# PreferredAI/PyBMF

Measured on AMD Instinct MI355X. Metric: MU iterations/sec (BinaryMF-Penalty, 100k x 20k Boolean, k=64), higher is better.
Workload: dtype i8 (bits x int8 digit planes on the integer MFMA, exact int32 accumulation); fp64 master factors and scalars; 1 GPU; BinaryMF-Penalty MU, 100000x20000 dense Boolean X, k=64, reg=1 growth=1.02, init normal+balance seed 2024; mae_pass=False, operands=i8x3, splits_xv=2, splits_xtu=11

## Files before the change

pybmf_amd/csrc/cover.hip:

```cpp
#include "common.h"

#include <algorithm>
#include <cstdlib>

namespace {

constexpr int RB = 8, NW = 8;
constexpr int CH = 256;

__global__ __launch_bounds__(512) void cover_kernel(const uint32_t* __restrict__ X, int64_t ldx, int64_t words,
                                                     const uint64_t* __restrict__ rowbits,
                                                     const uint32_t* __restrict__ colbits, int64_t ldcb, int kp,
                                                     int64_t rows_pad, int rows_per_block, int y_big, int rows_big,
                                                     unsigned long long* __restrict__ counts,
                                                     const int32_t* __restrict__ stop) {
    if (stop && *stop != 0) return;
    __shared__ __attribute__((aligned(16))) uint32_t vt[BMF_MAX_KP + 1][CH];
    const int lane = threadIdx.x & 63;
    const int wave = __builtin_amdgcn_readfirstlane(threadIdx.x >> 6);
    const int64_t w0 = (int64_t)blockIdx.x * CH;
    const int nw = (int)min((int64_t)CH, words - w0);

    {
        constexpr int PIECES = BMF_MAX_KP * CH / 4;
#pragma unroll
        for (int base = 0; base < PIECES; base += 4 * 512) {
            u32x4 v[4];
#pragma unroll
            for (int q = 0; q < 4; ++q) {
                const int p = base + q * 512 + threadIdx.x;
                const int l = p / (CH / 4), pw = (p % (CH / 4)) * 4;
                v[q] = (l < kp && pw < nw) ? *reinterpret_cast<const u32x4*>(colbits + (int64_t)l * ldcb + w0 + pw)
                                           : u32x4{0u, 0u, 0u, 0u};
            }
#pragma unroll
            for (int q = 0; q < 4; ++q) {
                const int p = base + q * 512 + threadIdx.x;
                *reinterpret_cast<u32x4*>(&vt[p / (CH / 4)][(p % (CH / 4)) * 4]) = v[q];
            }
        }
        if (threadIdx.x < CH / 4) *reinterpret_cast<u32x4*>(&vt[BMF_MAX_KP][threadIdx.x * 4]) = u32x4{0u, 0u, 0u, 0u};
    }
    __syncthreads();

    const int by = (int)blockIdx.y;
    const int64_t r0 = by < y_big ? (int64_t)by * rows_big : (int64_t)y_big * rows_big + (int64_t)(by - y_big) * rows_per_block;
    const int64_t r1 = min(r0 + (by < y_big ? rows_big : rows_per_block), rows_pad);
    if (r0 >= r1) return;
    const bool lane_on = 4 * lane < nw;
    unsigned tp = 0, fp = 0;
    const int nrows_wave = (int)((r1 - r0) / NW);
    const uint32_t* xw = X + (r0 + wave) * ldx + w0 + (lane_on ? 4 * lane : 0);
    const unsigned row_step = (unsigned)(NW * ldx);
    for (int g = 0; g < nrows_wave; g += 64) {
        const int jl = min(g + lane, nrows_wave - 1);
        const unsigned long long uvec = rowbits[r0 + wave + (int64_t)NW * jl];
        const unsigned uv_lo = (g + lane < nrows_wave) ? (unsigned)uvec : 0u;
        const unsigned uv_hi = (g + lane < nrows_wave) ? (unsigned)(uvec >> 32) : 0u;
        const int nj = min(64, nrows_wave - g);
        const uint32_t* xg = xw + (size_t)g * row_step;
        u32x4 x_cur[RB], x_nxt[RB];
#pragma unroll
        for (int b = 0; b < RB; ++b) x_cur[b] = *reinterpret_cast<const u32x4*>(xg + (size_t)b * row_step);
        for (int j0 = 0; j0 < nj; j0 += RB) {
            const int jn = (j0 + RB < nj) ? j0 + RB : j0;
#pragma unroll
            for (int b = 0; b < RB; ++b) x_nxt[b] = *reinterpret_cast<const u32x4*>(xg + (size_t)(jn + b) * row_step);
#pragma unroll
            for (int b = 0; b < RB; ++b) {
                unsigned ulo = __builtin_amdgcn_readlane(uv_lo, j0 + b);
                unsigned uhi = __builtin_amdgcn_readlane(uv_hi, j0 + b);
                if ((ulo | uhi) == 0u) continue;
                u32x4 pd = {0u, 0u, 0u, 0u};
                while (ulo | uhi) {
                    const int l0 = ulo ? __builtin_ctz(ulo) : BMF_MAX_KP;
                    ulo &= ulo - 1;
                    const int l1 = ulo ? __builtin_ctz(ulo) : BMF_MAX_KP;
                    ulo &= ulo - 1;
                    const int l2 = uhi ? 32 + __builtin_ctz(uhi) : BMF_MAX_KP;
                    uhi &= uhi - 1;
                    const int l3 = uhi ? 32 + __builtin_ctz(uhi) : BMF_MAX_KP;
                    uhi &= uhi - 1;
                    const u32x4 v0 = *reinterpret_cast<const u32x4*>(&vt[l0][4 * lane]);
                    const u32x4 v1 = *reinterpret_cast<const u32x4*>(&vt[l1][4 * lane]);
                    const u32x4 v2 = *reinterpret_cast<const u32x4*>(&vt[l2][4 * lane]);
                    const u32x4 v3 = *reinterpret_cast<const u32x4*>(&vt[l3][4 * lane]);
                    pd |= (v0 | v1) | (v2 | v3);
                }
                if (!lane_on) pd = u32x4{0u, 0u, 0u, 0u};
#pragma unroll
                for (int q = 0; q < 4; ++q) {
                    tp += __popc(x_cur[b][q] & pd[q]);
                    fp += __popc(~x_cur[b][q] & pd[q]);
                }
            }
#pragma unroll
            for (int b = 0; b < RB; ++b) x_cur[b] = x_nxt[b];
        }
    }
    __shared__ unsigned red[2][NW];
    tp = wave_sum(tp);
    fp = wave_sum(fp);
    if (lane == 0) { red[0][wave] = tp; red[1][wave] = fp; }
    __syncthreads();
    if (threadIdx.x < 2) {
        unsigned long long t = 0;
#pragma unroll
        for (int w = 0; w < NW; ++w) t += red[threadIdx.x][w];
        if (t) atomicAdd(&counts[threadIdx.x], t);
    }
}

template <int N4, int TW>
__global__ __launch_bounds__(1024) void cover_wide_kernel(const uint32_t* __restrict__ X, int64_t ldx, int64_t words, int chunk_words,
                                                           const uint64_t* __restrict__ rowbits, const uint32_t* __restrict__ colbits,
                                                           int64_t ldcb, int kp, int64_t rows_pad, int rows_per_block,
                                                           unsigned long long* __restrict__ counts, const int32_t* __restrict__ stop) {
    if (stop && *stop != 0) return;
    constexpr int CW = 256 * N4 + 64 * TW;
#ifndef BMF_COVER_RBW
#define BMF_COVER_RBW 2
#endif
    constexpr int NWV = 16, RBW = BMF_COVER_RBW;
    constexpr int NS = N4 + (TW ? 1 : 0);
    static_assert(BMF_MAX_KP * CW * 4 <= 160 * 1024 && (TW == 0 || TW == 2 || TW == 4) && NS >= 1, "chunk must fit the LDS");
    __shared__ __attribute__((aligned(16))) uint32_t vt[BMF_MAX_KP * CW];
    const int lane = threadIdx.x & 63;
    const int wave = __builtin_amdgcn_readfirstlane(threadIdx.x >> 6);
    const int64_t w0 = (int64_t)blockIdx.x * chunk_words;
    const int nw = (int)min((int64_t)min(CW, chunk_words), words - w0);

    {
        constexpr int PPC = CW / 4;
        constexpr int PIECES = BMF_MAX_KP * PPC;
        for (int base = 0; base < PIECES; base += 4 * 1024) {
            u32x4 v[4];
#pragma unroll
            for (int q = 0; q < 4; ++q) {
                const int p = base + q * 1024 + (int)threadIdx.x;
                const int l = p / PPC, pw = (p % PPC) * 4;
                v[q] = (p < PIECES && l < kp && pw < nw) ? *reinterpret_cast<const u32x4*>(colbits + (int64_t)l * ldcb + w0 + pw) : u32x4{0u, 0u, 0u, 0u};
            }
#pragma unroll
            for (int q = 0; q < 4; ++q) {
                const int p = base + q * 1024 + (int)threadIdx.x;
                if (p < PIECES) *reinterpret_cast<u32x4*>(&vt[4 * p]) = v[q];
            }
        }
    }
    __syncthreads();

    const int64_t r0 = (int64_t)blockIdx.y * rows_per_block;
    const int64_t r1 = min(r0 + rows_per_block, rows_pad);
    unsigned tp = 0, pp = 0;
    if (r0 < r1) {
        int soff[NS];
        bool son[NS];
#pragma unroll
        for (int sg = 0; sg < NS; ++sg) {
            const int wpl = (sg < N4) ? 4 : TW;
            const int o = 256 * sg + wpl * lane;
            son[sg] = o < nw;
            soff[sg] = son[sg] ? o : 0;
        }
        const int nrows_wave = (int)((r1 - r0) / NWV);
        const uint32_t* xw = X + (r0 + wave) * ldx + w0;
        const unsigned row_step = (unsigned)(NWV * ldx);
        for (int g = 0; g < nrows_wave; g += 64) {
            const int jl = min(g + lane, nrows_wave - 1);
            const unsigned long long uvec = rowbits[r0 + wave + (int64_t)NWV * jl];
            const unsigned uv_lo = (g + lane < nrows_wave) ? (unsigned)uvec : 0u;
            const unsigned uv_hi = (g + lane < nrows_wave) ? (unsigned)(uvec >> 32) : 0u;
            const int nj = min(64, nrows_wave - g);
            const uint32_t* xg = xw + (size_t)g * row_step;
            u32x4 x_cur[RBW][NS], x_nxt[RBW][NS];
            auto load_rows = [&](int j, u32x4 (&dst)[RBW][NS]) {
#pragma unroll
                for (int b = 0; b < RBW; ++b)
#pragma unroll
                    for (int sg = 0; sg < NS; ++sg) {
                        const uint32_t* p_ = xg + (size_t)(j + b) * row_step + soff[sg];
#ifdef BMF_COVER_PLAIN_LOADS
                        if (sg < N4 || TW == 4) dst[b][sg] = *reinterpret_cast<const u32x4*>(p_);
                        else {
                            const u32x2 t = *reinterpret_cast<const u32x2*>(p_);
                            dst[b][sg] = u32x4{t[0], t[1], 0u, 0u};
                        }
#else
                        if (sg < N4 || TW == 4) dst[b][sg] = __builtin_nontemporal_load(reinterpret_cast<const u32x4*>(p_));
                        else {
                            const u32x2 t = __builtin_nontemporal_load(reinterpret_cast<const u32x2*>(p_));
                            dst[b][sg] = u32x4{t[0], t[1], 0u, 0u};
                        }
#endif
                    }
            };
            load_rows(0, x_cur);
            for (int j0 = 0; j0 < nj; j0 += RBW) {
                const int jn = (j0 + RBW < nj) ? j0 + RBW : j0;
                load_rows(jn, x_nxt);
#pragma unroll
                for (int b = 0; b < RBW; ++b) {
                    const unsigned ulo = __builtin_amdgcn_readlane(uv_lo, j0 + b);
                    const unsigned uhi = __builtin_amdgcn_readlane(uv_hi, j0 + b);
                    unsigned long long u = ((unsigned long long)uhi << 32) | ulo;
                    if (u == 0ull) continue;
                    u32x4 pd[NS];
#pragma unroll
                    for (int sg = 0; sg < NS; ++sg) pd[sg] = u32x4{0u, 0u, 0u, 0u};
                    while (u) {
                        const int l0 = __builtin_ctzll(u);
                        u &= u - 1;
                        const int l1 = u ? __builtin_ctzll(u) : l0;
                        u &= u - 1;
                        const uint32_t* c0 = vt + l0 * CW;
                        const uint32_t* c1 = vt + l1 * CW;
#pragma unroll
                        for (int sg = 0; sg < NS; ++sg) {
                            if (sg < N4 || TW == 4) {
                                const u32x4 v0 = *reinterpret_cast<const u32x4*>(c0 + soff[sg]);
                                const u32x4 v1 = *reinterpret_cast<const u32x4*>(c1 + soff[sg]);
                                pd[sg] |= v0 | v1;
                            } else {
                                const u32x2 v0 = *reinterpret_cast<const u32x2*>(c0 + soff[sg]);
                                const u32x2 v1 = *reinterpret_cast<const u32x2*>(c1 + soff[sg]);
                                pd[sg][0] |= v0[0] | v1[0];
                                pd[sg][1] |= v0[1] | v1[1];
                            }
                        }
                    }
#pragma unroll
                    for (int sg = 0; sg < NS; ++sg) {
                        const int nq = (sg < N4 || TW == 4) ? 4 : 2;
#pragma unroll
                        for (int q = 0; q < 4; ++q)
                            if (q < nq) {
                                const unsigned pw_ = son[sg] ? pd[sg][q] : 0u;
                                tp += __popc(x_cur[b][sg][q] & pw_);
                                pp += __popc(pw_);
                            }
                    }
                }
#pragma unroll
                for (int b = 0; b < RBW; ++b)
#pragma unroll
                    for (int sg = 0; sg < NS; ++sg) x_cur[b][sg] = x_nxt[b][sg];
            }
        }
    }
    tp = wave_sum(tp);
    pp = wave_sum(pp);
    __syncthreads();
    if (lane == 0) { vt[wave] = tp; vt[NWV + wave] = pp; }
    __syncthreads();
    if (threadIdx.x < 2) {
        unsigned long long t = 0, a_ = 0;
#pragma unroll
        for (int w = 0; w < NWV; ++w) { t += vt[w]; a_ += vt[NWV + w]; }
        const unsigned long long val = threadIdx.x == 0 ? t : a_ - t;
        if (val) atomicAdd(&counts[threadIdx.x], val);
    }
}

__global__ __launch_bounds__(1024) void cover_delta_kernel(const uint32_t* __restrict__ X, int64_t ldx, int64_t words, int chunk_words,
                                                            const uint64_t* __restrict__ rowbits, const uint64_t* __restrict__ rowbits_prev,
                                                            const uint32_t* __restrict__ colbits, int64_t ldcb, int kp, int64_t rows_pad,
                                                            int rows_per_block, unsigned long long* __restrict__ counts,
                                                            const uint64_t* __restrict__ copy_src, uint64_t* __restrict__ copy_dst, int64_t copy_n,
                                                            const int32_t* __restrict__ stop) {
    if (stop && *stop != 0) return;
    constexpr int CW = 640, NWV = 16, NS = 3;
    __shared__ __attribute__((aligned(16))) uint32_t vt[BMF_MAX_KP * CW];
    const int lane = threadIdx.x & 63;
    const int wave = __builtin_amdgcn_readfirstlane(threadIdx.x >> 6);
    const int64_t w0 = (int64_t)blockIdx.x * chunk_words;
    const int nw = (int)min((int64_t)chunk_words, words - w0);
    const int64_t r0 = (int64_t)blockIdx.y * rows_per_block;
    const int64_t r1 = min(r0 + rows_per_block, rows_pad);

    if (copy_n > 0) {
        const int64_t nthreads = (int64_t)gridDim.x * gridDim.y * 1024;
        for (int64_t i = ((int64_t)blockIdx.y * gridDim.x + blockIdx.x) * 1024 + threadIdx.x; i < copy_n; i += nthreads) copy_dst[i] = copy_src[i];
    }

    unsigned long long need = 0ull;
    for (int64_t r = r0 + threadIdx.x; r < r1; r += 1024) {
        const unsigned long long a_ = rowbits[r], b_ = rowbits_prev[r];
        if (a_ != b_) need |= a_ | b_;
    }
    if (threadIdx.x < 2) vt[threadIdx.x] = 0u;
    __syncthreads();
    if (need) {
        atomicOr(&vt[0], (unsigned)need);
        atomicOr(&vt[1], (unsigned)(need >> 32));
    }
    __syncthreads();
    need = ((unsigned long long)vt[1] << 32) | vt[0];
    __syncthreads();
    if (need == 0ull) return;

    {
        constexpr int PPC = CW / 4;
        constexpr int PIECES = BMF_MAX_KP * PPC;
        const int nneed = __builtin_popcountll(need);
        if (nneed <= 12) {
            const int slot = (int)threadIdx.x / PPC, pw = ((int)threadIdx.x % PPC) * 4;
            u32x4 v[2];
            int col[2];
#pragma unroll
            for (int q = 0; q < 2; ++q) {
                unsigned long long m_ = need;
                for (int i = 0; i < 6 * q + slot && m_; ++i) m_ &= m_ - 1;
                col[q] = (slot < 6 && m_) ? __builtin_ctzll(m_) : -1;
                v[q] = (col[q] >= 0 && col[q] < kp && pw < nw) ? *reinterpret_cast<const u32x4*>(colbits + (int64_t)col[q] * ldcb + w0 + pw) : u32x4{0u, 0u, 0u, 0u};
            }
#pragma unroll
            for (int q = 0; q < 2; ++q)
                if (col[q] >= 0) *reinterpret_cast<u32x4*>(&vt[col[q] * CW + pw]) = v[q];
        } else {
            for (int base = 0; base < PIECES; base += 5 * 1024) {
                u32x4 v[5];
#pragma unroll
                for (int q = 0; q < 5; ++q) {
                    const int p = base + q * 1024 + (int)threadIdx.x;
                    const int l = p / PPC, pw = (p % PPC) * 4;
                    v[q] = (l < kp && pw < nw) ? *reinterpret_cast<const u32x4*>(colbits + (int64_t)l * ldcb + w0 + pw) : u32x4{0u, 0u, 0u, 0u};
                }
#pragma unroll
                for (int q = 0; q < 5; ++q) *reinterpret_cast<u32x4*>(&vt[4 * (base + q * 1024 + (int)threadIdx.x)]) = v[q];
            }
        }
    }
    __syncthreads();

    int soff[NS];
    bool son[NS];
#pragma unroll
    for (int sg = 0; sg < NS; ++sg) {
        const int o = 256 * sg + (sg < 2 ? 4 : 2) * lane;
        son[sg] = o < nw;
        soff[sg] = son[sg] ? o : 0;
    }
    const int nseg = (nw + 255) / 256;

    auto add_product = [&](unsigned long long u, u32x4 (&pd)[NS]) {
        while (u) {
            const int l0 = __builtin_ctzll(u);
            u &= u - 1;
            const int l1 = u ? __builtin_ctzll(u) : l0;
            u &= u - 1;
            const uint32_t* c0 = vt + l0 * CW;
            const uint32_t* c1 = vt + l1 * CW;
#pragma unroll
            for (int sg = 0; sg < NS; ++sg) {
                if (sg >= nseg) continue;
                if (sg < 2) {
                    pd[sg] |= *reinterpret_cast<const u32x4*>(c0 + soff[sg]) | *reinterpret_cast<const u32x4*>(c1 + soff[sg]);
                } else {
                    const u32x2 v0 = *reinterpret_cast<const u32x2*>(c0 + soff[sg]);
                    const u32x2 v1 = *reinterpret_cast<const u32x2*>(c1 + soff[sg]);
                    pd[sg][0] |= v0[0] | v1[0];
                    pd[sg][1] |= v0[1] | v1[1];
                }
            }
        }
#pragma unroll
        for (int sg = 0; sg < NS; ++sg)
            if (!son[sg]) pd[sg] = u32x4{0u, 0u, 0u, 0u};
    };

    constexpr int SCAN = 8;
    unsigned tpn = 0, tpo = 0, ppn = 0, ppo = 0;
    const int nrows = (int)(r1 - r0);
    const uint32_t* xb = X + r0 * ldx + w0;
    int rank0 = 0;
    for (int base = 0; base < nrows; base += 64 * SCAN) {
        unsigned long long un[SCAN], uo[SCAN];
#pragma unroll
        for (int g = 0; g < SCAN; ++g) {
            const int row = min(base + 64 * g + lane, nrows - 1);
            un[g] = rowbits[r0 + row];
            uo[g] = rowbits_prev[r0 + row];
        }
        int l_row = 0, l_nlo = 0, l_nhi = 0, l_olo = 0, l_ohi = 0, cnt = 0;
#pragma unroll
        for (int g = 0; g < SCAN; ++g) {
            const bool d_ = base + 64 * g < nrows && un[g] != uo[g];
            const unsigned long long mask = __ballot(d_);
            const int rk = rank0 + (int)__builtin_amdgcn_mbcnt_hi((unsigned)(mask >> 32), __builtin_amdgcn_mbcnt_lo((unsigned)mask, 0u));
            unsigned long long mine = __ballot(d_ && (rk & (NWV - 1)) == wave);
            rank0 += __builtin_popcountll(mask);
            while (mine) {
                const int j = __builtin_ctzll(mine);
                mine &= mine - 1;
                const bool slot = lane == cnt;
                l_row = slot ? base + 64 * g + j : l_row;
                l_nlo = slot ? __builtin_amdgcn_readlane((int)(unsigned)un[g], j) : l_nlo;
                l_nhi = slot ? __builtin_amdgcn_readlane((int)(unsigned)(un[g] >> 32), j) : l_nhi;
                l_olo = slot ? __builtin_amdgcn_readlane((int)(unsigned)uo[g], j) : l_olo;
                l_ohi = slot ? __builtin_amdgcn_readlane((int)(unsigned)(uo[g] >> 32), j) : l_ohi;
                ++cnt;
            }
        }
        if (cnt == 0) continue;
        u32x4 x_cur[NS], x_nxt[NS];
        auto load_row = [&](int t, u32x4 (&dst)[NS]) {
            const uint32_t* xr = xb + (int64_t)__builtin_amdgcn_readlane(l_row, t) * ldx;
#pragma unroll
            for (int sg = 0; sg < NS; ++sg) {
                dst[sg] = u32x4{0u, 0u, 0u, 0u};
                if (sg >= nseg) continue;
                if (sg < 2) dst[sg] = __builtin_nontemporal_load(reinterpret_cast<const u32x4*>(xr + soff[sg]));
                else {
                    const u32x2 v = __builtin_nontemporal_load(reinterpret_cast<const u32x2*>(xr + soff[sg]));
                    dst[sg] = u32x4{v[0], v[1], 0u, 0u};
                }
            }
        };
        load_row(0, x_cur);
        for (int t = 0; t < cnt; ++t) {
            load_row(t + 1 < cnt ? t + 1 : t, x_nxt);
            const unsigned wn_lo = __builtin_amdgcn_readlane(l_nlo, t), wn_hi = __builtin_amdgcn_readlane(l_nhi, t);
            const unsigned wo_lo = __builtin_amdgcn_readlane(l_olo, t), wo_hi = __builtin_amdgcn_readlane(l_ohi, t);
            const unsigned long long wn = ((unsigned long long)wn_hi << 32) | wn_lo, wo = ((unsigned long long)wo_hi << 32) | wo_lo;
            u32x4 pn[NS], po[NS];
#pragma unroll
            for (int sg = 0; sg < NS; ++sg) pn[sg] = u32x4{0u, 0u, 0u, 0u};
            add_product(wn & wo, pn);
#pragma unroll
            for (int sg = 0; sg < NS; ++sg) po[sg] = pn[sg];
            add_product(wn & ~wo, pn);
            add_product(wo & ~wn, po);
#pragma unroll
            for (int sg = 0; sg < NS; ++sg)
#pragma unroll
                for (int q = 0; q < 4; ++q) {
                    tpn += __popc(x_cur[sg][q] & pn[sg][q]);
                    tpo += __popc(x_cur[sg][q] & po[sg][q]);
                    ppn += __popc(pn[sg][q]);
                    ppo += __popc(po[sg][q]);
                }
#pragma unroll
            for (int sg = 0; sg < NS; ++sg) x_cur[sg] = x_nxt[sg];
        }
    }
    int tp = (int)wave_sum(tpn - tpo);
    int pp = (int)wave_sum(ppn - ppo);
    __syncthreads();
    if (lane == 0) { vt[wave] = (unsigned)tp; vt[NWV + wave] = (unsigned)pp; }
    __syncthreads();
    if (threadIdx.x < 2) {
        long long t = 0, a_ = 0;
#pragma unroll
        for (int w = 0; w < NWV; ++w) { t += (int)vt[w]; a_ += (int)vt[NWV + w]; }
        const long long val = threadIdx.x == 0 ? t : a_ - t;
        if (val) atomicAdd(&counts[threadIdx.x], (unsigned long long)val);
    }
}

__global__ __launch_bounds__(256) void product_bits_kernel(const uint64_t* __restrict__ rowbits, int64_t rows,
                                                            const uint32_t* __restrict__ colbits, int64_t ldcb, int64_t words,
                                                            uint32_t* __restrict__ out, int64_t ldo) {
    const int64_t total = rows * words;
    for (int64_t idx = (int64_t)blockIdx.x * 256 + threadIdx.x; idx < total; idx += (int64_t)gridDim.x * 256) {
        const int64_t row = idx / words, w = idx - row * words;
        unsigned long long u = rowbits[row];
        unsigned pd = 0u;
        while (u) {
            const int l = __builtin_ctzll(u);
            u &= u - 1;
            pd |= colbits[(int64_t)l * ldcb + w];
        }
        out[row * ldo + w] = pd;
    }
}

__global__ __launch_bounds__(256) void confusion_rows_kernel(const uint32_t* __restrict__ G, int64_t ldg,
                                                              const uint32_t* __restrict__ P, int64_t ldp, int64_t rows,
                                                              int64_t words, uint32_t* __restrict__ tp,
                                                              uint32_t* __restrict__ fp) {
    const int lane = threadIdx.x & 63;
    const int64_t nwaves = (int64_t)gridDim.x * 4;
    for (int64_t r = (int64_t)blockIdx.x * 4 + (threadIdx.x >> 6); r < rows; r += nwaves) {
        unsigned a = 0u, b = 0u;
        for (int64_t w = lane; w < words; w += 64) {
            const uint32_t g = G[r * ldg + w], p = P[r * ldp + w];
            a += __popc(g & p);
            b += __popc(~g & p);
        }
        a = wave_sum(a);
        b = wave_sum(b);
        if (lane == 0) {
            tp[r] = a;
            fp[r] = b;
        }
    }
}

}

extern "C" int bmf_confusion_rows(const uint32_t* Gbits, int64_t ldg, const uint32_t* Pbits, int64_t ldp, int64_t rows,
                                  int64_t words, uint32_t* tp, uint32_t* fp, void* stream) {
    BMF_REQUIRE(Gbits && Pbits && tp && fp, "bmf_confusion_rows: null pointer");
    BMF_REQUIRE(rows >= 1 && words >= 1 && ldg >= words && ldp >= words, "bmf_confusion_rows: bad shape");
    const int64_t blocks = (rows + 3) / 4;
    BMF_LAUNCH(confusion_rows_kernel, dim3((unsigned)(blocks < 4096 ? blocks : 4096)), dim3(256), 0, (hipStream_t)stream, Gbits, ldg,
               Pbits, ldp, rows, words, tp, fp);
    BMF_LAUNCH_CHECK();
    return BMF_OK;
}

namespace {
template <int N4, int TW>
void launch_cover_wide(dim3 grid, hipStream_t s, const uint32_t* Xbits, int64_t ldx, int64_t words, int chunk_words, const uint64_t* rowbits,
                       const uint32_t* colbits, int64_t ldcb, int kp, int64_t rows_pad, int rows_per_block, unsigned long long* counts,
                       const int32_t* stop) {
    BMF_LAUNCH((cover_wide_kernel<N4, TW>), grid, dim3(1024), 0, s, Xbits, ldx, words, chunk_words, rowbits, colbits, ldcb, kp, rows_pad,
               rows_per_block, counts, stop);
}
}

int bmf_cover_launch(const uint32_t* Xbits, int64_t rows_pad, int64_t ldx, int64_t words, const uint64_t* rowbits,
                     const uint32_t* colbits, int64_t ldcb, int kp, unsigned long long* counts, const int32_t* stop,
                     hipStream_t s) {
    if (words >= 128) {
        const int chunks_w = (int)((words + 639) / 640);
        int cw = (int)(((words + chunks_w - 1) / chunks_w + 127) / 128 * 128);
        const int n4 = cw / 256 > 2 ? 2 : cw / 256, rem = cw - 256 * n4;
        const int tw = rem == 0 ? 0 : (rem <= 128 ? 2 : 4);
        const int cus = bmf_cu_count_current();
        int64_t groups = cus / chunks_w > 0 ? cus / chunks_w : 1;
        const int64_t units = rows_pad / 64;
        if (groups > units) groups = units;
        const int rows_per_block = (int)(((units + groups - 1) / groups) * 64);
        groups = (rows_pad + rows_per_block - 1) / rows_per_block;
        dim3 grid((unsigned)chunks_w, (unsigned)groups);
        bool launched = false;
#define BMF_CW_CASE(N4_, TW_) \
    if (n4 == N4_ && tw == TW_) { launch_cover_wide<N4_, TW_>(grid, s, Xbits, ldx, words, cw, rowbits, colbits, ldcb, kp, rows_pad, rows_per_block, counts, stop); launched = true; }
        BMF_CW_CASE(0, 2) BMF_CW_CASE(0, 4) BMF_CW_CASE(1, 0) BMF_CW_CASE(1, 2) BMF_CW_CASE(1, 4) BMF_CW_CASE(2, 0) BMF_CW_CASE(2, 2)
#undef BMF_CW_CASE
        BMF_REQUIRE(launched, "bmf_cover_count: no kernel for chunks of %d words (segments %d, tail %d) at words=%lld", cw, n4, tw, (long long)words);
        BMF_LAUNCH_CHECK();
        return BMF_OK;
    }
    const unsigned chunks = (unsigned)((words + CH - 1) / CH);
    int64_t groups = 512 / chunks > 0 ? 512 / chunks : 1;
    int64_t units = rows_pad / 64;
    if (groups > units) groups = units;
    const double share = 0.63;
    int y_big = 0, rows_big = 0, rows_per_block;
    if (share > 0.5 && groups >= 8 && units >= 4 * groups) {
        y_big = (int)(groups / 2);
        const int64_t u_big = (int64_t)(share * 2.0 * (double)units / (double)groups + 0.999);
        rows_big = (int)(u_big * 64);
        const int64_t rest = units - std::min<int64_t>(units, (int64_t)y_big * u_big);
        const int64_t n_small = groups - y_big;
        rows_per_block = (int)(std::max<int64_t>(1, (rest + n_small - 1) / n_small) * 64);
    } else {
        rows_per_block = (int)(((units + groups - 1) / groups) * 64);
        groups = (rows_pad + rows_per_block - 1) / rows_per_block;
    }
    dim3 grid(chunks, (unsigned)groups), block(512);
    BMF_LAUNCH(cover_kernel, grid, block, 0, s, Xbits, ldx, words, rowbits, colbits, ldcb, kp, rows_pad,
                       rows_per_block, y_big, rows_big, counts, stop);
    BMF_LAUNCH_CHECK();
    return BMF_OK;
}

extern "C" int bmf_cover_count(const uint32_t* Xbits, int64_t rows_pad, int64_t ldx, int64_t words,
                               const uint64_t* rowbits, const uint32_t* colbits, int64_t ldcb, int kp,
                               unsigned long long* counts, const int32_t* stop, void* stream) {
    BMF_REQUIRE(Xbits && rowbits && colbits && counts, "bmf_cover_count: null pointer");
    BMF_REQUIRE(rows_pad > 0 && rows_pad % 64 == 0, "bmf_cover_count: rows_pad must be a positive multiple of 64");
    BMF_REQUIRE(words > 0 && words % 4 == 0 && ldx >= words && ldx % 4 == 0, "bmf_cover_count: words/ldx must be multiples of 4, ldx >= words");
    BMF_REQUIRE(ldcb >= words && ldcb % 4 == 0, "bmf_cover_count: ldcb must be >= words and a multiple of 4");
    BMF_REQUIRE(bmf_aligned16(colbits), "bmf_cover_count: colbits must be 16-byte aligned");
    BMF_REQUIRE(kp >= 1 && kp <= BMF_MAX_KP, "bmf_cover_count: kp must be 1..64");
    BMF_REQUIRE(bmf_aligned16(Xbits), "bmf_cover_count: Xbits must be 16-byte aligned");
    return bmf_cover_launch(Xbits, rows_pad, ldx, words, rowbits, colbits, ldcb, kp, counts, stop, (hipStream_t)stream);
}

int bmf_cover_delta_launch(const uint32_t* bits, int64_t ld, int64_t words, int64_t rows_pad, const uint64_t* rowbits,
                           const uint64_t* rowbits_prev, const uint32_t* colbits, int64_t ldcb, int kp, unsigned long long* counts,
                           const uint64_t* copy_src, uint64_t* copy_dst, int64_t copy_n, const int32_t* stop, hipStream_t s) {
    const int chunks_w = (int)((words + 639) / 640);
    const int64_t per = (words + chunks_w - 1) / chunks_w;
    const int cw = (int)(words >= 128 ? (per + 127) / 128 * 128 : words);
    const int cus = bmf_cu_count_current();
    int64_t groups = cus / chunks_w > 0 ? cus / chunks_w : 1;
    const int64_t units = rows_pad / 64;
    if (groups > units) groups = units;
    const int rows_per_block = (int)(((units + groups - 1) / groups) * 64);
    groups = (rows_pad + rows_per_block - 1) / rows_per_block;
    BMF_LAUNCH(cover_delta_kernel, dim3((unsigned)chunks_w, (unsigned)groups), dim3(1024), 0, s, bits, ld, words, cw, rowbits, rowbits_prev, colbits,
               ldcb, kp, rows_pad, rows_per_block, counts, copy_src, copy_dst, copy_n, stop);
    BMF_LAUNCH_CHECK();
    return BMF_OK;
}

extern "C" int bmf_cover_delta(const uint32_t* bits, int64_t ld, int64_t words, int64_t rows_pad, const uint64_t* rowbits,
                               const uint64_t* rowbits_prev, const uint32_t* colbits, int64_t ldcb, int kp, unsigned long long* counts,
                               const uint64_t* copy_src, uint64_t* copy_dst, int64_t copy_n, const int32_t* stop, void* stream) {
    BMF_REQUIRE(bits && rowbits && rowbits_prev && colbits && counts, "bmf_cover_delta: null pointer");
    BMF_REQUIRE(rows_pad > 0 && rows_pad % 64 == 0, "bmf_cover_delta: rows_pad must be a positive multiple of 64");
    BMF_REQUIRE(words >= 4 && words % 4 == 0 && ld >= words && ld % 4 == 0, "bmf_cover_delta: words/ld must be multiples of 4, ld >= words >= 4");
    BMF_REQUIRE(ldcb >= words && ldcb % 4 == 0, "bmf_cover_delta: ldcb must be >= words and a multiple of 4");
    BMF_REQUIRE(bmf_aligned16(bits) && bmf_aligned16(colbits), "bmf_cover_delta: bits and colbits must be 16-byte aligned");
    BMF_REQUIRE(kp >= 1 && kp <= BMF_MAX_KP, "bmf_cover_delta: kp must be 1..64");
    BMF_REQUIRE(copy_n >= 0 && (copy_n == 0 || (copy_src && copy_dst)), "bmf_cover_delta: copy_n > 0 needs copy_src and copy_dst");
    BMF_REQUIRE(copy_n == 0 || (copy_dst != rowbits && copy_dst != rowbits_prev), "bmf_cover_delta: the copy must not overwrite the words this launch compares");
    return bmf_cover_delta_launch(bits, ld, words, rows_pad, rowbits, rowbits_prev, colbits, ldcb, kp, counts, copy_src, copy_dst, copy_n, stop,
                                  (hipStream_t)stream);
}

extern "C" int bmf_boolean_product_bits(const uint64_t* rowbits, int64_t rows, const uint32_t* colbits, int64_t ldcb, int kp,
                                        int64_t words, uint32_t* out, int64_t ldo, void* stream) {
    BMF_REQUIRE(rowbits && colbits && out, "bmf_boolean_product_bits: null pointer");
    BMF_REQUIRE(rows > 0 && words > 0 && ldcb >= words && ldo >= words, "bmf_boolean_product_bits: bad shape");
    BMF_REQUIRE(kp >= 1 && kp <= BMF_MAX_KP, "bmf_boolean_product_bits: kp must be 1..64");
    const int64_t blocks = (rows * words + 255) / 256;
    BMF_LAUNCH(product_bits_kernel, dim3((unsigned)(blocks < 8192 ? blocks : 8192)), dim3(256), 0, (hipStream_t)stream,
                       rowbits, rows, colbits, ldcb, words, out, ldo);
    BMF_LAUNCH_CHECK();
    return BMF_OK;
}
```

Before: 1929 iterations/s.

## Pipeline changed-row X loads through a ring buffer with buffer loads in cover_delta

Replaces the single-row prefetch in cover_delta_kernel with a RING-deep (default 4) register ring of raw buffer loads whose out-of-range bounds return zeros. This removes the per-segment masking logic. The block-level need mask is now reduced with DPP wave ORs through LDS instead of shared atomics and an extra barrier. Deeper prefetch is meant to hide global-memory latency on the scattered changed rows, at the cost of more VGPRs per lane, which can lower occupancy at 1024 threads per block.

```diff
diff --git a/pybmf_amd/csrc/cover.hip b/pybmf_amd/csrc/cover.hip
--- a/pybmf_amd/csrc/cover.hip
+++ b/pybmf_amd/csrc/cover.hip
@@ -262,6 +262,18 @@
     }
 }
 
+#ifndef BMF_COVER_RING
+#define BMF_COVER_RING 4
+#endif
+__device__ __forceinline__ unsigned wave_or(unsigned v) {
+    v |= (unsigned)__builtin_amdgcn_update_dpp(0, (int)v, 0xB1, 0xF, 0xF, false);
+    v |= (unsigned)__builtin_amdgcn_update_dpp(0, (int)v, 0x4E, 0xF, 0xF, false);
+    v |= (unsigned)__builtin_amdgcn_update_dpp(0, (int)v, 0x141, 0xF, 0xF, false);
+    v |= (unsigned)__builtin_amdgcn_update_dpp(0, (int)v, 0x140, 0xF, 0xF, false);
+    return (unsigned)(__builtin_amdgcn_readlane((int)v, 0) | __builtin_amdgcn_readlane((int)v, 16) | __builtin_amdgcn_readlane((int)v, 32) |
+                      __builtin_amdgcn_readlane((int)v, 48));
+}
+
 __global__ __launch_bounds__(1024) void cover_delta_kernel(const uint32_t* __restrict__ X, int64_t ldx, int64_t words, int chunk_words,
                                                             const uint64_t* __restrict__ rowbits, const uint64_t* __restrict__ rowbits_prev,
                                                             const uint32_t* __restrict__ colbits, int64_t ldcb, int kp, int64_t rows_pad,
@@ -269,7 +281,7 @@
                                                             const uint64_t* __restrict__ copy_src, uint64_t* __restrict__ copy_dst, int64_t copy_n,
                                                             const int32_t* __restrict__ stop) {
     if (stop && *stop != 0) return;
-    constexpr int CW = 640, NWV = 16, NS = 3;
+    constexpr int CW = 640, NWV = 16;
     __shared__ __attribute__((aligned(16))) uint32_t vt[BMF_MAX_KP * CW];
     const int lane = threadIdx.x & 63;
     const int wave = __builtin_amdgcn_readfirstlane(threadIdx.x >> 6);
@@ -283,23 +295,25 @@
         for (int64_t i = ((int64_t)blockIdx.y * gridDim.x + blockIdx.x) * 1024 + threadIdx.x; i < copy_n; i += nthreads) copy_dst[i] = copy_src[i];
     }
 
+    const int nrows = (int)(r1 - r0);
+    if (nrows <= 0) return;
+
     unsigned long long need = 0ull;
-    for (int64_t r = r0 + threadIdx.x; r < r1; r += 1024) {
-        const unsigned long long a_ = rowbits[r], b_ = rowbits_prev[r];
-        if (a_ != b_) need |= a_ | b_;
-    }
-    if (threadIdx.x < 2) vt[threadIdx.x] = 0u;
-    __syncthreads();
-    if (need) {
-        atomicOr(&vt[0], (unsigned)need);
-        atomicOr(&vt[1], (unsigned)(need >> 32));
-    }
-    __syncthreads();
-    need = ((unsigned long long)vt[1] << 32) | vt[0];
-    __syncthreads();
-    if (need == 0ull) return;
-
     {
+        unsigned long long need_l = 0ull;
+        for (int64_t r = r0 + threadIdx.x; r < r1; r += 1024) {
+            const unsigned long long a_ = rowbits[r], b_ = rowbits_prev[r];
+            if (a_ != b_) need_l |= a_ | b_;
+        }
+        const unsigned lo = wave_or((unsigned)need_l), hi = wave_or((unsigned)(need_l >> 32));
+        if (lane == 0) { vt[2 * wave] = lo; vt[2 * wave + 1] = hi; }
+        __syncthreads();
+        const unsigned w_ = lane < 2 * NWV ? vt[lane] : 0u;
+        need = ((unsigned long long)wave_or((lane & 1) ? w_ : 0u) << 32) | wave_or((lane & 1) ? 0u : w_);
+        if (need == 0ull) return;
+    }
+
+    auto fill = [&](unsigned long long need) {
         constexpr int PPC = CW / 4;
         constexpr int PIECES = BMF_MAX_KP * PPC;
         const int nneed = __builtin_popcountll(need);
@@ -330,20 +344,13 @@
                 for (int q = 0; q < 5; ++q) *reinterpret_cast<u32x4*>(&vt[4 * (base + q * 1024 + (int)threadIdx.x)]) = v[q];
             }
         }
-    }
-    __syncthreads();
-
-    int soff[NS];
-    bool son[NS];
-#pragma unroll
-    for (int sg = 0; sg < NS; ++sg) {
-        const int o = 256 * sg + (sg < 2 ? 4 : 2) * lane;
-        son[sg] = o < nw;
-        soff[sg] = son[sg] ? o : 0;
-    }
+    };
+
+    const int soff0 = 4 * lane, soff1 = 256 + 4 * lane, soff2 = 512 + 2 * lane;
     const int nseg = (nw + 255) / 256;
-
-    auto add_product = [&](unsigned long long u, u32x4 (&pd)[NS]) {
+    struct RowWords { u32x4 a, b; u32x2 c; };
+
+    auto add_product = [&](unsigned long long u, RowWords& pd) {
         while (u) {
             const int l0 = __builtin_ctzll(u);
             u &= u - 1;
@@ -351,28 +358,20 @@
             u &= u - 1;
             const uint32_t* c0 = vt + l0 * CW;
             const uint32_t* c1 = vt + l1 * CW;
-#pragma unroll
-            for (int sg = 0; sg < NS; ++sg) {
-                if (sg >= nseg) continue;
-                if (sg < 2) {
-                    pd[sg] |= *reinterpret_cast<const u32x4*>(c0 + soff[sg]) | *reinterpret_cast<const u32x4*>(c1 + soff[sg]);
-                } else {
-                    const u32x2 v0 = *reinterpret_cast<const u32x2*>(c0 + soff[sg]);
-                    const u32x2 v1 = *reinterpret_cast<const u32x2*>(c1 + soff[sg]);
-                    pd[sg][0] |= v0[0] | v1[0];
-                    pd[sg][1] |= v0[1] | v1[1];
-                }
-            }
-        }
-#pragma unroll
-        for (int sg = 0; sg < NS; ++sg)
-            if (!son[sg]) pd[sg] = u32x4{0u, 0u, 0u, 0u};
+            pd.a |= *reinterpret_cast<const u32x4*>(c0 + soff0) | *reinterpret_cast<const u32x4*>(c1 + soff0);
+            if (nseg > 1) pd.b |= *reinterpret_cast<const u32x4*>(c0 + soff1) | *reinterpret_cast<const u32x4*>(c1 + soff1);
+            if (nseg > 2) pd.c |= *reinterpret_cast<const u32x2*>(c0 + soff2) | *reinterpret_cast<const u32x2*>(c1 + soff2);
+        }
     };
 
-    constexpr int SCAN = 8;
+    constexpr int SCAN = 8, RING = BMF_COVER_RING;
+    static_assert(RING >= 1 && 64 * SCAN / NWV + RING <= 64, "the list and the ring slots past its end must fit the 64 lanes");
     unsigned tpn = 0, tpo = 0, ppn = 0, ppo = 0;
-    const int nrows = (int)(r1 - r0);
     const uint32_t* xb = X + r0 * ldx + w0;
+    __syncthreads();
+    fill(need);
+    __builtin_amdgcn_s_waitcnt(0x0F70);
+    __syncthreads();
     int rank0 = 0;
     for (int base = 0; base < nrows; base += 64 * SCAN) {
         unsigned long long un[SCAN], uo[SCAN];
@@ -402,46 +401,58 @@
                 ++cnt;
             }
         }
-        if (cnt == 0) continue;
-        u32x4 x_cur[NS], x_nxt[NS];
-        auto load_row = [&](int t, u32x4 (&dst)[NS]) {
+        RowWords x[RING];
+        auto load_row = [&](int t, RowWords& dst) {
             const uint32_t* xr = xb + (int64_t)__builtin_amdgcn_readlane(l_row, t) * ldx;
-#pragma unroll
-            for (int sg = 0; sg < NS; ++sg) {
-                dst[sg] = u32x4{0u, 0u, 0u, 0u};
-                if (sg >= nseg) continue;
-                if (sg < 2) dst[sg] = __builtin_nontemporal_load(reinterpret_cast<const u32x4*>(xr + soff[sg]));
-                else {
-                    const u32x2 v = __builtin_nontemporal_load(reinterpret_cast<const u32x2*>(xr + soff[sg]));
-                    dst[sg] = u32x4{v[0], v[1], 0u, 0u};
-                }
-            }
+            const auto rsrc = __builtin_amdgcn_make_buffer_rsrc(const_cast<uint32_t*>(xr), 0, t < cnt ? 4 * nw : 0, 0x00020000);
+            dst.a = __builtin_amdgcn_raw_buffer_load_b128(rsrc, 4 * soff0, 0, 2);
+            dst.b = __builtin_amdgcn_raw_buffer_load_b128(rsrc, 4 * soff1, 0, 2);
+            dst.c = __builtin_amdgcn_raw_buffer_load_b64(rsrc, 4 * soff2, 0, 2);
         };
-        load_row(0, x_cur);
-        for (int t = 0; t < cnt; ++t) {
-            load_row(t + 1 < cnt ? t + 1 : t, x_nxt);
+        auto count_row = [&](int t, const RowWords& xr) {
             const unsigned wn_lo = __builtin_amdgcn_readlane(l_nlo, t), wn_hi = __builtin_amdgcn_readlane(l_nhi, t);
             const unsigned wo_lo = __builtin_amdgcn_readlane(l_olo, t), wo_hi = __builtin_amdgcn_readlane(l_ohi, t);
             const unsigned long long wn = ((unsigned long long)wn_hi << 32) | wn_lo, wo = ((unsigned long long)wo_hi << 32) | wo_lo;
-            u32x4 pn[NS], po[NS];
-#pragma unroll
-            for (int sg = 0; sg < NS; ++sg) pn[sg] = u32x4{0u, 0u, 0u, 0u};
+            RowWords pn = {u32x4{0u, 0u, 0u, 0u}, u32x4{0u, 0u, 0u, 0u}, u32x2{0u, 0u}};
             add_product(wn & wo, pn);
-#pragma unroll
-            for (int sg = 0; sg < NS; ++sg) po[sg] = pn[sg];
+            RowWords po = pn;
             add_product(wn & ~wo, pn);
             add_product(wo & ~wn, po);
 #pragma unroll
-            for (int sg = 0; sg < NS; ++sg)
-#pragma unroll
-                for (int q = 0; q < 4; ++q) {
-                    tpn += __popc(x_cur[sg][q] & pn[sg][q]);
-                    tpo += __popc(x_cur[sg][q] & po[sg][q]);
-                    ppn += __popc(pn[sg][q]);
-                    ppo += __popc(po[sg][q]);
+            for (int q = 0; q < 4; ++q) {
+                tpn += __popc(xr.a[q] & pn.a[q]) + __popc(xr.b[q] & pn.b[q]);
+                tpo += __popc(xr.a[q] & po.a[q]) + __popc(xr.b[q] & po.b[q]);
+                ppn += __popc(pn.a[q]) + __popc(pn.b[q]);
+                ppo += __popc(po.a[q]) + __popc(po.b[q]);
+            }
+#pragma unroll
+            for (int q = 0; q < 2; ++q) {
+                tpn += __popc(xr.c[q] & pn.c[q]);
+                tpo += __popc(xr.c[q] & po.c[q]);
+                ppn += __popc(pn.c[q]);
+                ppo += __popc(po.c[q]);
+            }
+        };
+        if (cnt > RING) {
+#pragma unroll
+            for (int d = 0; d < RING; ++d) {
+                load_row(d, x[d]);
+                __builtin_amdgcn_sched_barrier(0);
+            }
+            for (int t0 = 0; t0 < cnt; t0 += RING) {
+#pragma unroll
+                for (int d = 0; d < RING; ++d) {
+                    if (t0 + d < cnt) count_row(t0 + d, x[d]);
+                    load_row(t0 + d + RING, x[d]);
                 }
-#pragma unroll
-            for (int sg = 0; sg < NS; ++sg) x_cur[sg] = x_nxt[sg];
+            }
+        } else if (cnt > 0) {
+            load_row(0, x[0]);
+            for (int t = 0; t < cnt; ++t) {
+                load_row(t + 1, x[1]);
+                count_row(t, x[0]);
+                x[0] = x[1];
+            }
         }
     }
     int tp = (int)wave_sum(tpn - tpo);
```

After: 1925 iterations/s. No clear change (-0.2%).
